# pvrohin/Structure-from-Motion-

Measured on AMD Instinct MI355X. Metric: BA LM-iterations/sec (+ RANSAC hypotheses/sec, final reproj RMSE vs ref), higher is better.
Workload: dtype f64; 1 GPU; cfg5: BA 200 cams / 500000 pts / 4000000 obs, Schur-complement LM, points sharded over 1 rank(s); parallelism=point-shard x1 + RCCL all-reduce of the reduced camera system

## Files before the change

### structure-from-motion-_amd/csrc/ba.hip

```cpp
#include <rccl/rccl.h>

#include <algorithm>
#include <chrono>
#include <condition_variable>
#include <deque>
#include <functional>
#include <mutex>
#include <thread>
#include <cmath>
#include <cstdio>
#include <cstdlib>
#include <cstring>
#include <memory>
#include <utility>
#include <numeric>
#include <vector>

#include "sfm_common.hpp"
#include "sfm_geom.hpp"
#include "host_pool.hpp"

struct LocalGroup {
    int nranks = 0;
    std::mutex mu;
// ... 30 lines not shown

__device__ __forceinline__ double clampd(double x) { return fmin(fmax(x, 1e-6), 1e32); }

__device__ __forceinline__ double wave_sum(double v) {
#pragma unroll
    for (int o = 32; o > 0; o >>= 1) v += __shfl_xor(v, o);
    return v;
}

template <int NV>
__device__ __forceinline__ void block_sum_store(double (&v)[NV], double *out) {
    __shared__ double red[PT_THREADS / 64][NV];
    const int lane = threadIdx.x & 63, w = threadIdx.x >> 6;
#pragma unroll
    for (int k = 0; k < NV; ++k) {
        const double s = wave_sum(v[k]);
        if (lane == 0) red[w][k] = s;
    }
    __syncthreads();
    if (threadIdx.x == 0) {
#pragma unroll
        for (int k = 0; k < NV; ++k) {
            double s = 0;
            for (int i = 0; i < PT_THREADS / 64; ++i) s += red[i][k];
            out[k] = s;
        }
    }
}

constexpr int GS_STRIDE = 32;
constexpr int GS_WORDS = 9 * GS_STRIDE;

template <int NV, int NT = PT_THREADS>
__device__ __forceinline__ void grid_sum_last(double (&v)[NV], double *partial, unsigned *counter, double *out) {
    __shared__ double red[NT / 64][NV];
    __shared__ int last;
    const int lane = threadIdx.x & 63, w = threadIdx.x >> 6;
    const unsigned nblk = gridDim.x;
#pragma unroll
    for (int k = 0; k < NV; ++k) {
        const double s = wave_sum(v[k]);
        if (lane == 0) red[w][k] = s;
    }
    __syncthreads();
    if (threadIdx.x == 0) {
#pragma unroll
        for (int k = 0; k < NV; ++k) {
            double s = 0;
            for (int i = 0; i < NT / 64; ++i) s += red[i][k];
            __hip_atomic_store(partial + (int64_t)NV * blockIdx.x + k, s, __ATOMIC_RELAXED, __HIP_MEMORY_SCOPE_AGENT);
        }
        asm volatile("s_waitcnt vmcnt(0)" ::: "memory");
        const unsigned g = blockIdx.x % 8, ng = (nblk - g + 7) / 8, ngroups = nblk < 8 ? nblk : 8;
        int l = 0;
        if (__hip_atomic_fetch_add(counter + GS_STRIDE * (1 + g), 1u, __ATOMIC_RELAXED, __HIP_MEMORY_SCOPE_AGENT) ==
            ng - 1)
            l = __hip_atomic_fetch_add(counter, 1u, __ATOMIC_RELAXED, __HIP_MEMORY_SCOPE_AGENT) == ngroups - 1;
        last = l;
    }
    __syncthreads();
    if (!last) return;
    __shared__ double tot[NV][NT];
    double s[NV];
#pragma unroll
    for (int k = 0; k < NV; ++k) s[k] = 0;
    constexpr int GS_BATCH = NV > 1 ? 8 : 16;
    for (unsigned b0 = threadIdx.x; b0 < nblk; b0 += GS_BATCH * NT) {
        double v16[NV][GS_BATCH];
#pragma unroll
        for (int u = 0; u < GS_BATCH; ++u) {
            const unsigned b = b0 + u * NT;
#pragma unroll
            for (int k = 0; k < NV; ++k)
                v16[k][u] = b < nblk ? __hip_atomic_load(partial + (int64_t)NV * b + k, __ATOMIC_RELAXED,
                                                         __HIP_MEMORY_SCOPE_AGENT)
                                     : 0.0;
        }
#pragma unroll
        for (int k = 0; k < NV; ++k)
#pragma unroll
            for (int u = 0; u < GS_BATCH; ++u) s[k] += v16[k][u];
    }
#pragma unroll
    for (int k = 0; k < NV; ++k) tot[k][threadIdx.x] = s[k];
    __syncthreads();
    for (int st = NT / 2; st > 0; st >>= 1) {
        if ((int)threadIdx.x < st)
#pragma unroll
            for (int k = 0; k < NV; ++k) tot[k][threadIdx.x] += tot[k][threadIdx.x + st];
        __syncthreads();
    }
    if (threadIdx.x < NV) out[threadIdx.x] = tot[threadIdx.x][0];
    if (threadIdx.x < 9) __hip_atomic_store(counter + GS_STRIDE * threadIdx.x, 0u, __ATOMIC_RELAXED, __HIP_MEMORY_SCOPE_AGENT);
}


__device__ __forceinline__ void obs_model(const double *__restrict__ Rt, const double *X, const double (&K)[9],
                                          double2 ob, double (&r)[2], double (&A)[2][3], double (&p)[3]) {
#pragma unroll
    for (int i = 0; i < 3; ++i) p[i] = Rt[3 * i] * X[0] + Rt[3 * i + 1] * X[1] + Rt[3 * i + 2] * X[2];
    const double xc0 = p[0] + Rt[9], xc1 = p[1] + Rt[10], xc2 = p[2] + Rt[11];
    double u[3];
#pragma unroll
    for (int i = 0; i < 3; ++i) u[i] = K[3 * i] * xc0 + K[3 * i + 1] * xc1 + K[3 * i + 2] * xc2;
    const double iw = 1.0 / (u[2] + 1e-8);
    const double pu = u[0] * iw, pv = u[1] * iw;
    r[0] = ob.x - pu;
    r[1] = ob.y - pv;
#pragma unroll
    for (int c = 0; c < 3; ++c) {
        A[0][c] = -(iw * K[c] - pu * iw * K[6 + c]);
        A[1][c] = -(iw * K[3 + c] - pv * iw * K[6 + c]);
    }
}

__device__ __forceinline__ void obs_Ap(const double *__restrict__ Rt, const double *X, const double (&K)[9],
                                       double (&A)[2][3], double (&p)[3]) {
#pragma unroll
    for (int i = 0; i < 3; ++i) p[i] = Rt[3 * i] * X[0] + Rt[3 * i + 1] * X[1] + Rt[3 * i + 2] * X[2];
    const double xc0 = p[0] + Rt[9], xc1 = p[1] + Rt[10], xc2 = p[2] + Rt[11];
    double u[3];
#pragma unroll
    for (int i = 0; i < 3; ++i) u[i] = K[3 * i] * xc0 + K[3 * i + 1] * xc1 + K[3 * i + 2] * xc2;
    const double iw = 1.0 / (u[2] + 1e-8);
    const double pu = u[0] * iw, pv = u[1] * iw;
#pragma unroll
// ... 2 lines not shown
        A[1][c] = -(iw * K[3 + c] - pv * iw * K[6 + c]);
    }
}

__device__ __forceinline__ void jc_of(const double (&A)[2][3], const double (&p)[3], double (&Jc)[2][6]) {
#pragma unroll
    for (int a = 0; a < 2; ++a) {
        Jc[a][0] = A[a][1] * (-p[2]) + A[a][2] * p[1];
        Jc[a][1] = A[a][0] * p[2] + A[a][2] * (-p[0]);
        Jc[a][2] = A[a][0] * (-p[1]) + A[a][1] * p[0];
        Jc[a][3] = A[a][0];
        Jc[a][4] = A[a][1];
        Jc[a][5] = A[a][2];
    }
}

__device__ __forceinline__ double obs_cost(const double *__restrict__ Rt, const double *X, const double (&K)[9],
                                           double2 ob) {
    double xc[3];
#pragma unroll
    for (int i = 0; i < 3; ++i) xc[i] = Rt[3 * i] * X[0] + Rt[3 * i + 1] * X[1] + Rt[3 * i + 2] * X[2] + Rt[9 + i];
    double u[3];
#pragma unroll
    for (int i = 0; i < 3; ++i) u[i] = K[3 * i] * xc[0] + K[3 * i + 1] * xc[1] + K[3 * i + 2] * xc[2];
    const double iw = 1.0 / (u[2] + 1e-8);
    const double r0 = ob.x - u[0] * iw, r1 = ob.y - u[1] * iw;
    return 0.5 * (r0 * r0 + r1 * r1);
}

struct Kmat {
    double k[9];
};

template <int G>
__global__ void __launch_bounds__(PT_THREADS) k_linearize(int64_t np_, const int32_t *__restrict__ pstart,
                                                          const int32_t *__restrict__ cam,
                                                          const double2 *__restrict__ obs, Kmat Km,
                                                          const double *__restrict__ Rt,
                                                          const double *__restrict__ X,
                                                          double *__restrict__ Vg, double *__restrict__ partial,
                                                          unsigned *__restrict__ counter, double *__restrict__ cost_out,
                                                          int want_cost, const int *__restrict__ gate, double gtol,
                                                          unsigned *__restrict__ nbig) {
    if (gate && !*gate) return;
    const int64_t gt = (int64_t)blockIdx.x * PT_THREADS + threadIdx.x;
    const int64_t p = gt / G;
    const int sub = (int)(gt % G);
    double K[9];
#pragma unroll
    for (int i = 0; i < 9; ++i) K[i] = Km.k[i];
    double acc[1] = {0.0};
    double V[6] = {0, 0, 0, 0, 0, 0}, g[3] = {0, 0, 0};
    if (p < np_) {
        double x[3] = {X[3 * p], X[3 * p + 1], X[3 * p + 2]};
        for (int32_t o = pstart[p] + sub; o < pstart[p + 1]; o += G) {
            const double *Rt_c = Rt + 12 * cam[o];
            double r[2], A[2][3], q[3];
            obs_model(Rt_c, x, K, obs[o], r, A, q);
            double Jp[2][3];
#pragma unroll
            for (int a = 0; a < 2; ++a)
#pragma unroll
                for (int c = 0; c < 3; ++c) Jp[a][c] = A[a][0] * Rt_c[c] + A[a][1] * Rt_c[3 + c] + A[a][2] * Rt_c[6 + c];
            acc[0] += 0.5 * (r[0] * r[0] + r[1] * r[1]);
            V[0] += Jp[0][0] * Jp[0][0] + Jp[1][0] * Jp[1][0];
            V[1] += Jp[0][0] * Jp[0][1] + Jp[1][0] * Jp[1][1];
            V[2] += Jp[0][0] * Jp[0][2] + Jp[1][0] * Jp[1][2];
            V[3] += Jp[0][1] * Jp[0][1] + Jp[1][1] * Jp[1][1];
            V[4] += Jp[0][1] * Jp[0][2] + Jp[1][1] * Jp[1][2];
            V[5] += Jp[0][2] * Jp[0][2] + Jp[1][2] * Jp[1][2];
#pragma unroll
            for (int i = 0; i < 3; ++i) g[i] += Jp[0][i] * r[0] + Jp[1][i] * r[1];
        }
    }
#pragma unroll
    for (int i = 0; i < 6; ++i) V[i] = group_sum<G>(V[i]);
#pragma unroll
    for (int i = 0; i < 3; ++i) g[i] = group_sum<G>(g[i]);
    if (p < np_ && sub == 0) {
        double *vg = Vg + 9 * p;
#pragma unroll
        for (int i = 0; i < 6; ++i) vg[i] = V[i];
#pragma unroll
        for (int i = 0; i < 3; ++i) vg[6 + i] = g[i];
    }
    if (gtol > 0.0) {
        int big = 0;
        if (p < np_ && sub == 0)
#pragma unroll
            for (int i = 0; i < 3; ++i) big += fabs(g[i]) >= gtol;
#pragma unroll
        for (int o = 32; o > 0; o >>= 1) big += __shfl_xor(big, o);
        if ((threadIdx.x & 63) == 0 && big) atomicAdd(nbig, (unsigned)big);
    }
    if (want_cost) grid_sum_last<1>(acc, partial, counter, cost_out);
}

constexpr int LIN_PRE = 4;
constexpr int LIN_CL_THREADS = 256;
#ifndef SFM_LIN_CAM_STRIDE
#define SFM_LIN_CAM_STRIDE 14
#endif
constexpr int LIN_CAM = SFM_LIN_CAM_STRIDE;
template <int G, int NT = LIN_CL_THREADS>
__global__ void __launch_bounds__(NT) k_linearize_cl(int64_t np_, int32_t nc, const int32_t *__restrict__ pstart,
                                                     const int32_t *__restrict__ cam, const double2 *__restrict__ obs,
                                                     Kmat Km, const double *__restrict__ Rt,
                                                     const double *__restrict__ X, double *__restrict__ Vg,
                                                     double *__restrict__ partial, unsigned *__restrict__ counter,
                                                     double *__restrict__ cost_out, int want_cost,
                                                     const int *__restrict__ gate, double gtol,
                                                     unsigned *__restrict__ nbig) {
    if (gate && !*gate) return;
    struct Pre {
        int32_t o0, o1;
        double x[3];
    };
    auto fetch = [&](int64_t g, Pre &P) {
        const int64_t p = g / G;
        const bool live = p < np_;
        P.o0 = live ? pstart[p] : 0;
        P.o1 = live ? pstart[p + 1] : 0;
#pragma unroll
        for (int i = 0; i < 3; ++i) P.x[i] = live ? X[3 * p + i] : 0.0;
    };
    const int64_t stride = (int64_t)gridDim.x * NT;
    Pre cur;
    fetch((int64_t)blockIdx.x * NT + threadIdx.x, cur);
    extern __shared__ __attribute__((aligned(16))) double lin_cam[];
#pragma unroll 4
    for (int i = threadIdx.x; i < 12 * nc; i += NT) lin_cam[LIN_CAM * (i / 12) + i % 12] = Rt[i];
    __syncthreads();
    double K[9];
#pragma unroll
    for (int i = 0; i < 9; ++i) K[i] = Km.k[i];
    double acc[1] = {0.0};
    int big = 0;
    for (int64_t gt = (int64_t)blockIdx.x * NT + threadIdx.x; gt / G < np_; gt += stride) {
        const int64_t p = gt / G;
        const int sub = (int)(gt % G);
        const int32_t o0 = cur.o0, o1 = cur.o1;
        int32_t cpre[LIN_PRE];
        double2 opre[LIN_PRE];
#pragma unroll
        for (int k = 0; k < LIN_PRE; ++k) {
            const int32_t o = o0 + sub + k * G;
            cpre[k] = o < o1 ? cam[o] : 0;
            opre[k] = o < o1 ? obs[o] : make_double2(0.0, 0.0);
        }
        Pre nxt;
        fetch(gt + stride, nxt);
        const double x[3] = {cur.x[0], cur.x[1], cur.x[2]};
        double V[6] = {0, 0, 0, 0, 0, 0}, g[3] = {0, 0, 0};
        auto add = [&](int32_t c, double2 ob) {
            const double *Rt_c = lin_cam + LIN_CAM * c;
            double r[2], A[2][3], q[3];
            obs_model(Rt_c, x, K, ob, r, A, q);
            double Jp[2][3];
#pragma unroll
            for (int a = 0; a < 2; ++a)
#pragma unroll
                for (int c2 = 0; c2 < 3; ++c2)
                    Jp[a][c2] = A[a][0] * Rt_c[c2] + A[a][1] * Rt_c[3 + c2] + A[a][2] * Rt_c[6 + c2];
            acc[0] += 0.5 * (r[0] * r[0] + r[1] * r[1]);
            V[0] += Jp[0][0] * Jp[0][0] + Jp[1][0] * Jp[1][0];
            V[1] += Jp[0][0] * Jp[0][1] + Jp[1][0] * Jp[1][1];
            V[2] += Jp[0][0] * Jp[0][2] + Jp[1][0] * Jp[1][2];
            V[3] += Jp[0][1] * Jp[0][1] + Jp[1][1] * Jp[1][1];
            V[4] += Jp[0][1] * Jp[0][2] + Jp[1][1] * Jp[1][2];
            V[5] += Jp[0][2] * Jp[0][2] + Jp[1][2] * Jp[1][2];
#pragma unroll
            for (int i = 0; i < 3; ++i) g[i] += Jp[0][i] * r[0] + Jp[1][i] * r[1];
        };
#pragma unroll
        for (int k = 0; k < LIN_PRE; ++k)
            if (o0 + sub + k * G < o1) add(cpre[k], opre[k]);
        for (int32_t o = o0 + sub + LIN_PRE * G; o < o1; o += G) add(cam[o], obs[o]);
#pragma unroll
        for (int i = 0; i < 6; ++i) V[i] = group_sum<G>(V[i]);
#pragma unroll
        for (int i = 0; i < 3; ++i) g[i] = group_sum<G>(g[i]);
        if (sub == 0) {
            double *vg = Vg + 9 * p;
#pragma unroll
            for (int i = 0; i < 6; ++i) vg[i] = V[i];
#pragma unroll
            for (int i = 0; i < 3; ++i) vg[6 + i] = g[i];
            if (gtol > 0.0)
#pragma unroll
                for (int i = 0; i < 3; ++i) big += fabs(g[i]) >= gtol;
        }
        cur = nxt;
    }
    if (gtol > 0.0) {
#pragma unroll
        for (int o = 32; o > 0; o >>= 1) big += __shfl_xor(big, o);
        if ((threadIdx.x & 63) == 0 && big) atomicAdd(nbig, (unsigned)big);
    }
    if (want_cost) grid_sum_last<1, NT>(acc, partial, counter, cost_out);
}

constexpr int OBS_THREADS = 256;

__global__ void __launch_bounds__(OBS_THREADS) k_point_prep(int64_t np_, const double *__restrict__ Vg,
                                                            const double *__restrict__ lam, double *__restrict__ Lq,
                                                            const int *__restrict__ gate) {
    if (gate && !*gate) return;
    __shared__ double buf[9 * OBS_THREADS];
    const int64_t p0 = (int64_t)blockIdx.x * OBS_THREADS;
    const int n9 = 9 * (int)(np_ - p0 < OBS_THREADS ? np_ - p0 : OBS_THREADS);
    const int t = threadIdx.x;
#pragma unroll
    for (int k = 0; k < 9; ++k)
        if (t + k * OBS_THREADS < n9) buf[t + k * OBS_THREADS] = Vg[9 * p0 + t + k * OBS_THREADS];
    __syncthreads();
    if (9 * t < n9) {
        const double lambda = *lam;
        double *vg = buf + 9 * t;
        const double v00 = vg[0] + lambda * clampd(vg[0]), v01 = vg[1], v02 = vg[2];
        const double v11 = vg[3] + lambda * clampd(vg[3]), v12 = vg[4];
// ... 1201 lines not shown
        chain_fetch<TB>(ob, A, nsp, nT - 2, lane);
        double acc = 0;
        lds_barrier();
        int kt = nT - 1;
        for (; kt >= 1; kt -= 2) {
            chain_step<TB>(oa, A, nsp, kt, x, acc, lane, li);
            chain_step<TB>(ob, A, nsp, kt - 1, x, acc, lane, li);
        }
        if (kt == 0) chain_step<TB>(oa, A, nsp, 0, x, acc, lane, li);
    } else {
        const int r = t - 64;
        double la[TB], lb[TB];
        rows_fetch<TB>(la, A, nsp, nT - 1, r);
        rows_fetch<TB>(lb, A, nsp, nT - 2, r);
        lds_barrier();
        int kt = nT - 1;
        for (; kt >= 1; kt -= 2) {
            rows_step<TB>(la, A, nsp, kt, x, r);
            rows_step<TB>(lb, A, nsp, kt - 1, x, r);
        }
        if (kt == 0) rows_step<TB>(la, A, nsp, 0, x, r);
    }
    lds_barrier();
    for (int i = t; i < nsp; i += SOLVE_THREADS) xg[i] = x[i];
    if (ct.nc > 0) {
        __shared__ double red[3][SOLVE_THREADS];
        camera_trial<SOLVE_THREADS>(ct.nc, x, ct.payload, ct.ns, *ct.lam, ct.Rt, ct.Rt_new, ct.cam_out, red);
    }
}

struct LMState {
    double lambda, nu, cost, cost0;
    int status, accepted, iters, done;
    int run_lin, run_step, accept_now, pad;
    double spec_lambda;
    int armed;
    int use_spec;
    int run_real;
    int run_spec;
};

struct HostLM {
    LMState st;
    int seq, pad[3];
};
constexpr int kHostRing = 4;

__global__ void __launch_bounds__(256) k_gather_cam_major(int64_t no, const int32_t *__restrict__ pt,
                                                         const double2 *__restrict__ obs, int32_t *cm_pt,
                                                         double2 *__restrict__ cm_obs) {
    const int64_t k = (int64_t)blockIdx.x * 256 + threadIdx.x;
    if (k >= no) return;
    const int32_t o = cm_pt[k];
    cm_pt[k] = pt[o];
    cm_obs[k] = obs[o];
}

__global__ void k_lm_reset(LMState *lm, double lambda0, int *bad) {
    lm->lambda = lambda0; lm->nu = 2.0; lm->cost = 0.0; lm->cost0 = 0.0;
    lm->status = 4; lm->accepted = 0; lm->iters = 0; lm->done = 0;
    lm->run_lin = 1; lm->run_step = 1; lm->accept_now = 0; lm->pad = 0;
    lm->spec_lambda = lambda0 * 2.0; lm->armed = 0; lm->use_spec = 0; lm->run_real = 1; lm->run_spec = 0;
    bad[0] = 0;
}

__global__ void k_lm_init(LMState *lm, const double *lin_cost) {
    const double c0 = *lin_cost;
    lm->cost = lm->cost0 = c0;
    if (!isfinite(c0)) {
        lm->status = 6;
        lm->done = 1;
        lm->run_step = 0;
        lm->run_lin = 0;
        lm->run_real = 0;
        lm->run_spec = 0;
    }
}

__device__ __forceinline__ LMState lm_decide(LMState lm, const double *__restrict__ h, int bad, int max_iterations,
                                             int fixed, double ftol, double ptol, double lambda0, int spec) {
#pragma clang fp contract(off)
    if (lm.done) { lm.accept_now = 0; return lm; }
    const bool built = (spec & 2) && lm.run_spec;
    const double built_lambda = lm.spec_lambda;
    const double cost = lm.cost;
    const double cost_new = h[0];
    const double model = 0.5 * (h[1] + h[4]);
    const double dnorm = sqrt(h[2] + h[5]), xnorm = sqrt(h[3] + h[6]);
    const double rho = (!bad && model > 0) ? (cost - cost_new) / model : -1.0;
    lm.iters += 1;
    int done = 0;
    if (!bad && isfinite(cost_new) && rho > 1e-3) {
        lm.accept_now = 1;
        const double dcost = cost - cost_new;
// ... 46 lines not shown
    __shared__ int big;
    if (threadIdx.x == 0) big = 0;
    __syncthreads();
    int b = 0;
    for (int i = threadIdx.x; i < 6 * nc; i += blockDim.x) b += fabs(gbuf[1 + i]) >= gtol;
    if (b) atomicAdd(&big, b);
    __syncthreads();
    if (threadIdx.x == 0 && big == 0 && gbuf[0] == 0.0) {
        lm->status = 2;
        lm->done = 1;
        lm->run_step = 0;
        lm->run_lin = 0;
        lm->run_real = 0;
        lm->run_spec = 0;
    }
}

__global__ void k_lm_step(const LMState *__restrict__ lm_in, LMState *__restrict__ lm_out,
                          const double *__restrict__ h, const int *__restrict__ bad_in, int *__restrict__ bad_next,
                          int max_iterations, int fixed, double ftol, double ptol, double lambda0, int64_t np_,
                          int32_t nc, double *__restrict__ X, const double *__restrict__ X2, double *__restrict__ Rt,
                          const double *__restrict__ Rt2, HostLM *__restrict__ ring, int seq, int spec) {
    const LMState lm = lm_decide(*lm_in, h, *bad_in, max_iterations, fixed, ftol, ptol, lambda0, spec);
    if (blockIdx.x == 0 && threadIdx.x == 0) {
        *lm_out = lm;
        *bad_next = 0;
        if (ring) {
            HostLM *r = ring + (seq - 1) % kHostRing;
            r->st = lm;
            __hip_atomic_store(&r->seq, seq, __ATOMIC_RELEASE, __HIP_MEMORY_SCOPE_SYSTEM);
        }
    }
    if (!lm.accept_now) return;
    const int64_t i0 = (int64_t)blockIdx.x * blockDim.x + threadIdx.x, st = (int64_t)gridDim.x * blockDim.x;
    for (int64_t i = i0; i < 3 * np_; i += st) X[i] = X2[i];
    for (int64_t i = i0; i < 12 * (int64_t)nc; i += st) Rt[i] = Rt2[i];
}

constexpr int LIN_CL_LANES = 2;
constexpr int LIN_LANES = 4;
constexpr int BS_LANES = 2;

template <int TB>
static int launch_cholesky_t(const double *payload, int32_t ns, const double *lam, double *A, int32_t nsp, double *b,
                             double *D, int *bad, hipStream_t s, const int *gate, const CamTrialArgs &ct,
                             const SlabSrc &src, int dpp) {
    const int nT = nsp / TB;
    for (int st = 0; st < nT; ++st) {
        const int T = nT - st;
        const int extra = st >= 1 || src.slab ? 1 : 0;
        hipLaunchKernelGGL(k_chol_col<TB>, dim3(T * (T + 1) / 2 + extra), dim3(256), 0, s, A, nsp, st, D, b, bad,
                           payload, ns, lam, gate, dpp, st == 0 ? src : SlabSrc{nullptr, nullptr, 0, 0},
                           const_cast<double *>(payload));
        SFM_HIP(hipGetLastError());
    }
    hipLaunchKernelGGL(k_chol_backsolve<TB>, dim3(1), dim3(SOLVE_THREADS), 0, s, A, nsp, b,
                       D + ((nT - 1) & 1) * TB * TB, ct, gate);
    SFM_HIP(hipGetLastError());
    return 0;
}

static int launch_cholesky(const double *payload, int32_t ns, const double *lam, double *A, int32_t nsp, double *b,
                           double *D, int *bad, hipStream_t s, int tb, const int *gate, const CamTrialArgs &ct,
                           const SlabSrc &src, int dpp) {
    return tb == 32 ? launch_cholesky_t<32>(payload, ns, lam, A, nsp, b, D, bad, s, gate, ct, src, dpp)
                    : launch_cholesky_t<16>(payload, ns, lam, A, nsp, b, D, bad, s, gate, ct, src, dpp);
// ... 203 lines not shown
    case gjr::TREG:
        hipLaunchKernelGGL((gjr::k_gjr_solve<gjr::TREG, 0>), dim3(g.nT), dim3(gjr::THREADS), gjr::DYN_LDS, s, a);
        break;
    default:
        hipLaunchKernelGGL((gjr::k_gjr_solve<gjr::TREG_L, gjr::TLDS_L>), dim3(g.nT), dim3(gjr::THREADS), gjr::DYN_LDS,
                           s, a);
        break;
    }
    SFM_HIP(hipGetLastError());
    return 0;
}

constexpr int BS_PRE = 6;
#ifndef SFM_BS_CAM_STRIDE
#define SFM_BS_CAM_STRIDE 30
#endif
constexpr int BS_CAM = SFM_BS_CAM_STRIDE;
static_assert(BS_CAM >= 30, "Rt 12 | Rt_new 12 | dc 6");
constexpr int BS_CAM_LDS_MAX = 64 * 1024;
template <int G, bool CL, int NT = PT_THREADS>
__global__ void __launch_bounds__(NT) k_backsub_trial(int64_t np_, int32_t nc, const int32_t *__restrict__ pstart,
                                                              const int32_t *__restrict__ cam,
                                                              const double2 *__restrict__ obs, Kmat Km,
                                                              const double *__restrict__ Vg,
                                                              const double *__restrict__ Lq_own,
                                                              const double *__restrict__ Lq_spec,
                                                              const int *__restrict__ use_spec,
                                                              const double *__restrict__ dc, const double *__restrict__ lam,
                                                              const double *__restrict__ Rt,
                                                              const double *__restrict__ Rt_new,
                                                              const double *__restrict__ X,
                                                              double *__restrict__ X_new, double *__restrict__ partial,
                                                              unsigned *__restrict__ counter, double *__restrict__ out,
                                                              const int *__restrict__ gate) {
    if (gate && !*gate) return;
    const double lambda = *lam;
    const double *__restrict__ Lq = use_spec && *use_spec ? Lq_spec : Lq_own;
    double K[9];
#pragma unroll
    for (int i = 0; i < 9; ++i) K[i] = Km.k[i];
    double acc[4] = {0, 0, 0, 0};
    struct Pre {
        int32_t o0, o1;
        double x[3], g[3], dg[3], l[6];
    };
    auto fetch = [&](int64_t gtn, Pre &P) {
        const int64_t p = gtn / G;
        const bool live = p < np_;
        P.o0 = live ? pstart[p] : 0;
        P.o1 = live ? pstart[p + 1] : 0;
        const double *vg = Vg + 9 * (live ? p : 0);
        const double *l = Lq + 9 * (live ? p : 0);
#pragma unroll
        for (int i = 0; i < 3; ++i) {
            P.x[i] = live ? X[3 * p + i] : 0.0;
            P.g[i] = vg[6 + i];
        }
        P.dg[0] = vg[0];
        P.dg[1] = vg[3];
        P.dg[2] = vg[5];
#pragma unroll
        for (int i = 0; i < 6; ++i) P.l[i] = l[i];
    };
    const int64_t stride = (int64_t)gridDim.x * NT;
    Pre cur;
    fetch((int64_t)blockIdx.x * NT + threadIdx.x, cur);
    extern __shared__ __attribute__((aligned(16))) double bs_cam[];
    if constexpr (CL) {
// ... 48 lines not shown
    };
#pragma unroll
    for (int k = 0; k < BS_PRE; ++k)
        if (o0 + sub + k * G < o1) wt_add(cpre[k]);
    for (int32_t o = o0 + sub + BS_PRE * G; o < o1; o += G) wt_add(cam[o]);
#pragma unroll
    for (int i = 0; i < 3; ++i) wt[i] = group_sum<G>(wt[i]);
    if (live) {
        const double rhs[3] = {-cur.g[0] - wt[0], -cur.g[1] - wt[1], -cur.g[2] - wt[2]};
        const double *l = cur.l;
        const double y0 = l[0] * rhs[0];
        const double y1 = l[1] * rhs[0] + l[3] * rhs[1];
        const double y2 = l[2] * rhs[0] + l[4] * rhs[1] + l[5] * rhs[2];
        const double dp[3] = {l[0] * y0 + l[1] * y1 + l[2] * y2, l[3] * y1 + l[4] * y2, l[5] * y2};
        double xn[3];
#pragma unroll
        for (int i = 0; i < 3; ++i) xn[i] = x[i] + dp[i];
        if (sub == 0) {
#pragma unroll
            for (int i = 0; i < 3; ++i) {
                X_new[3 * p + i] = xn[i];
                acc[1] += dp[i] * (lambda * clampd(cur.dg[i]) * dp[i] - cur.g[i]);
                acc[2] += dp[i] * dp[i];
                acc[3] += x[i] * x[i];
            }
        }
#pragma unroll
        for (int k = 0; k < BS_PRE; ++k)
            if (o0 + sub + k * G < o1) acc[0] += obs_cost(cRn + RS * cpre[k], xn, K, opre[k]);
        for (int32_t o = o0 + sub + BS_PRE * G; o < o1; o += G) acc[0] += obs_cost(cRn + RS * cam[o], xn, K, obs[o]);
    }
    cur = nxt;
    }
    grid_sum_last<4, NT>(acc, partial, counter, out);
}

static void h_rotvec_to_R(const double *w, double *R) {
    double th2 = w[0] * w[0] + w[1] * w[1] + w[2] * w[2];
    double th = std::sqrt(th2), a, b;
    if (th < 1e-6) {
        a = 1.0 - th2 / 6.0 + th2 * th2 / 120.0;
        b = 0.5 - th2 / 24.0 + th2 * th2 / 720.0;
    } else {
        a = std::sin(th) / th;
        b = (1.0 - std::cos(th)) / th2;
    }
    double x = w[0], y = w[1], z = w[2];
    R[0] = 1.0 - b * (y * y + z * z); R[1] = -a * z + b * x * y;       R[2] = a * y + b * x * z;
    R[3] = a * z + b * x * y;         R[4] = 1.0 - b * (x * x + z * z); R[5] = -a * x + b * y * z;
    R[6] = -a * y + b * x * z;        R[7] = a * x + b * y * z;         R[8] = 1.0 - b * (x * x + y * y);
}

static void h_R_to_rotvec(const double *R, double *w) {
    double tr = R[0] + R[4] + R[8], q[4];
    if (tr > R[0] && tr > R[4] && tr > R[8]) {
        q[3] = 1.0 + tr;
        q[0] = R[7] - R[5]; q[1] = R[2] - R[6]; q[2] = R[3] - R[1];
    } else {
        int i = (R[0] >= R[4] && R[0] >= R[8]) ? 0 : (R[4] >= R[8] ? 1 : 2);
        int j = (i + 1) % 3, k = (j + 1) % 3;
        q[i] = 1.0 - tr + 2.0 * R[i * 4];
        q[j] = R[j * 3 + i] + R[i * 3 + j];
        q[k] = R[k * 3 + i] + R[i * 3 + k];
        q[3] = R[k * 3 + j] - R[j * 3 + k];
    }
    double nq = std::sqrt(q[0] * q[0] + q[1] * q[1] + q[2] * q[2] + q[3] * q[3]);
    for (double &v : q) v /= nq;
// ... 1120 lines not shown
    uint32_t *d_sw_pairs = nullptr;
    int2 *d_sw_blkij = nullptr;
    double2 *d_obs = nullptr;
    double *d_Rt = nullptr, *d_Rt2 = nullptr, *d_X = nullptr, *d_X2 = nullptr;
    double *d_Vg = nullptr, *d_Lq = nullptr;
    double *d_payload = nullptr, *d_A = nullptr, *d_b = nullptr, *d_D = nullptr;
    double *d_partial = nullptr, *d_scal = nullptr;
    int *d_bad = nullptr;
    int *d_sw_err = nullptr;
    unsigned *d_count = nullptr;
    unsigned *d_nbig = nullptr;
    double *d_gbuf = nullptr;
    double gtol = 0.0;
    HostLM *h_ring = nullptr, *d_ring = nullptr;
    bool timing = false;
    int64_t payload_len = 0;
    int pt_blocks = 0;
    int bs_cl_blocks = 0;
    int lin_cl_blocks = 0;
    hipEvent_t ev[2 * T_NT] = {};
    hipEvent_t ev_it[2 * T_NT * kEvSlots] = {};
    LMState *d_lm = nullptr;
    GjPlan gjp;
    GjBufs gjb;
    int gj_epoch = 0;
    GjrPlan gjrp;
    GjrBufs gjrb;
    unsigned gjr_tag = 0;
    bool gjr_fold = false;
    hipEvent_t ev_solve = nullptr;
    bool spec_ok = false;
    bool spec_on = false;
    bool spec_armed = false;
    SweepSplit sp_split = {};
    int32_t sp_free_cus = 0;
    int32_t *d_sp_split_of = nullptr;
    double *d_sp_slab = nullptr;
    double *d_sp_Lq[2] = {nullptr, nullptr}, *d_sp_payload[2] = {nullptr, nullptr};
    SpecKit sk;
    bool sp_queued[kEvSlots] = {};
    double t_acc[T_NT] = {};
    int t_iters = 0;
    std::vector<std::pair<void *, size_t>> allocs;
    ~sfm_ba_problem() {
        (void)hipSetDevice(device);
        if (ev_solve && comm && comm->local) {
            std::lock_guard<std::mutex> lk(comm->local->solve_mu);
            if (comm->local->last_solve == ev_solve) comm->local->last_solve = nullptr;
        }
        const bool idle = stream && hipStreamSynchronize(stream) == hipSuccess &&
                          (!sk.stream || hipStreamSynchronize(sk.stream) == hipSuccess);
        for (auto &a : allocs) {
            if (idle) pool_free(a.first, a.second, device);
            else (void)hipFree(a.first);
        }
        if (stream && idle) {
            kit_release(*this);
            return;
        }
        (void)hipGetLastError();
        if (h_ring) (void)hipHostFree(h_ring);
        for (auto &e : ev)
            if (e) (void)hipEventDestroy(e);
        for (auto &e : ev_it)
            if (e) (void)hipEventDestroy(e);
        if (ev_solve) (void)hipEventDestroy(ev_solve);
// ... 888 lines not shown
    if (!p->comm) return 0;
    if (p->comm->local) return p->comm->nranks > 1 ? local_allreduce(p, buf, n) : 0;
    ncclResult_t r = ncclAllReduce(buf, buf, (size_t)n, ncclDouble, ncclSum, p->comm->comm, p->stream);
    if (r != ncclSuccess) {
        set_error("ncclAllReduce: %s", ncclGetErrorString(r));
        return SFM_ERR_COMM;
    }
    return 0;
}

static CamLinArgs camlin_args(const sfm_ba_problem *p, bool fused, const int *glin) {
    CamLinArgs a;
    a.items = fused ? p->d_fitems : p->d_items;
    a.wg_first = fused ? p->d_fwg_first : p->d_wg_first;
    a.cm_pt = p->d_cm_pt;
    a.cm_obs = p->d_cm_obs;
    a.X = p->d_X;
    a.Rt = p->d_Rt;
    a.Km = p->K;
    a.slab2 = p->d_slab2;
    a.blocks = fused ? p->d_fblocks : p->d_blocks;
    a.nblocks = p->ndiag_blocks;
    a.nwg = fused ? p->cl_fused_wg : p->ndiag_items;
    a.direct = !fused && p->ndiag_items == p->ndiag_blocks;
    a.camlin = p->d_camlin;
    a.counter = p->d_count + 2 * GS_WORDS;
    a.glin = glin;
    return a;
}

static int run_linearize(sfm_ba_problem *p, int par, int want_cost) {
    hipStream_t s = p->stream;
    const int *glin = &p->d_lm[par].run_lin;

    if (p->lin_cl_blocks > 0) {
        const int nb = std::max(1, std::min(ceil_div(p->np * LIN_CL_LANES, LIN_CL_THREADS), p->lin_cl_blocks));
        hipLaunchKernelGGL(k_linearize_cl<LIN_CL_LANES>, dim3(nb), dim3(LIN_CL_THREADS), (size_t)8 * LIN_CAM * p->nc, s,
                           p->np, p->nc, p->d_pstart, p->d_cam, p->d_obs, p->K, p->d_Rt, p->d_X, p->d_Vg, p->d_partial,
                           p->d_count, p->d_scal + 8, want_cost, glin, p->gtol, p->d_nbig);
        SFM_HIP(hipGetLastError());
        if (p->ndiag_items && !p->cl_fused) {
            const CamLinArgs cl = camlin_args(p, false, glin);
            hipLaunchKernelGGL(k_camera_lin<256>, dim3(p->ndiag_items), dim3(256), 0, s, cl);
            SFM_HIP(hipGetLastError());
        }
        return want_cost ? allreduce(p, p->d_scal + 8, 1) : 0;
    }
    const int nbl = std::max(1, ceil_div(p->np * LIN_LANES, PT_THREADS));
    hipLaunchKernelGGL(k_linearize<LIN_LANES>, dim3(nbl), dim3(PT_THREADS), 0, s, p->np, p->d_pstart, p->d_cam,
                       p->d_obs, p->K, p->d_Rt, p->d_X, p->d_Vg, p->d_partial, p->d_count, p->d_scal + 8, want_cost,
                       glin, p->gtol, p->d_nbig);
    SFM_HIP(hipGetLastError());
    if (p->ndiag_items && !p->cl_fused) {
        const CamLinArgs cl = camlin_args(p, false, glin);
        hipLaunchKernelGGL(k_camera_lin<256>, dim3(p->ndiag_items), dim3(256), 0, s, cl);
        SFM_HIP(hipGetLastError());
    }
    return want_cost ? allreduce(p, p->d_scal + 8, 1) : 0;
}

static int run_spec_chain(sfm_ba_problem *p, int par, int it, bool timed) {
    hipStream_t s2 = p->sk.stream;
    const int *gsp = &p->d_lm[par].run_spec;
    const double *lam = &p->d_lm[par].spec_lambda;
    double *Lq = p->d_sp_Lq[it & 1], *payload = p->d_sp_payload[it & 1];
    hipEvent_t *tm = p->sk.tm + 4 * (it % kEvSlots);
    if (timed) SFM_HIP(hipEventRecord(tm[0], s2));
    hipLaunchKernelGGL(k_point_prep, dim3(std::max(1, ceil_div(p->np, OBS_THREADS))), dim3(OBS_THREADS), 0, s2,
                       (int64_t)p->np, p->d_Vg, lam, Lq, gsp);
    SFM_HIP(hipGetLastError());
    if (timed) SFM_HIP(hipEventRecord(tm[1], s2));
    if (timed) SFM_HIP(hipEventRecord(tm[2], s2));
    const SweepSplit &sp = p->sp_split;
    const int nsweep = sp.S                ? sp.nfull + p->sw_nrange * sp.nsplit * sp.S
                       : p->sw_nrange < NXCD ? NXCD * ceil_div(p->sw_nspec, NXCD / p->sw_nrange)
                                             : NXCD * p->sw_nspec * ceil_div(p->sw_nrange, NXCD);
    auto sweep_k = p->sw_pinhole ? k_schur_sweep<1, true> : k_schur_sweep<1>;
    hipLaunchKernelGGL(sweep_k, dim3(nsweep), dim3(SW_THREADS), p->sw_lds_bytes, s2, p->sw_nspec, p->sw_nrange,
                       p->sw_nbd, p->sw_L, p->d_sw_rchunk, p->d_sw_nload, p->d_sw_goff, p->d_sw_groups,
                       p->d_sw_lanegrp, p->d_sw_scam, reinterpret_cast<const uint32_t *>(p->d_sw_list), p->d_sw_pairs,
                       p->d_sw_hdr, p->d_X, Lq, p->d_Rt, p->K, p->d_sp_slab, gsp, p->sw_debug, nsweep,
                       camlin_args(p, true, &p->d_lm[par].run_lin), (long long *)nullptr, p->d_sw_err, sp);
    SFM_HIP(hipGetLastError());
    hipLaunchKernelGGL(k_schur_finish, dim3(ceil_div(p->sw_nbd * ITEM_W, FIN_THREADS)), dim3(FIN_THREADS), 0, s2, p->ns,
                       p->sw_nbd, p->sw_nrange, p->d_sw_blkij, p->d_sp_slab, p->d_camlin, payload, gsp,
                       p->d_sp_split_of, sp);
    SFM_HIP(hipGetLastError());
    if (timed) SFM_HIP(hipEventRecord(tm[3], s2));
    SFM_HIP(hipEventRecord(p->sk.join[it % kSpecRing], s2));
    p->sp_queued[it % kEvSlots] = true;
    return 0;
}

static int run_step(sfm_ba_problem *p, hipEvent_t *ev, int par, int it) {
    hipStream_t s = p->stream;
    int rc;
    const bool timed = ev != nullptr;
    const int *gst = &p->d_lm[par].run_step;
    const int *greal = p->spec_on ? &p->d_lm[par].run_real : gst;
    const int *use_spec = p->spec_on ? &p->d_lm[par].use_spec : nullptr;
    const double *Lq_spec = p->spec_on ? p->d_sp_Lq[(it - 1) & 1] : nullptr;
    const double *pay_spec = p->spec_on ? p->d_sp_payload[(it - 1) & 1] : nullptr;
    const double *lam = &p->d_lm[par].lambda;
    int *bad = p->d_bad + par;
    if (timed) SFM_HIP(hipEventRecord(ev[2 * T_PREP], s));
    hipLaunchKernelGGL(k_point_prep, dim3(std::max(1, ceil_div(p->np, OBS_THREADS))), dim3(OBS_THREADS), 0, s, (int64_t)p->np,
                       p->d_Vg, lam, p->d_Lq, greal);
    SFM_HIP(hipGetLastError());
    if (timed) SFM_HIP(hipEventRecord(ev[2 * T_PREP + 1], s));
    if (timed) SFM_HIP(hipEventRecord(ev[2 * T_SCHUR], s));
    const int nsweep = p->sw_split.S       ? p->sw_split.nfull + NXCD * p->sw_split.nsplit * p->sw_split.S
                       : p->sw_nrange < NXCD ? NXCD * ceil_div(p->sw_nspec, NXCD / p->sw_nrange)
                                             : NXCD * p->sw_nspec * ceil_div(p->sw_nrange, NXCD);
    const bool fused = p->cl_fused && p->ndiag_items;
    auto sweep_k = p->sw_pinhole ? k_schur_sweep<1, true> : k_schur_sweep<1>;
    hipLaunchKernelGGL(sweep_k, dim3(nsweep + (fused ? p->cl_fused_wg : 0)), dim3(SW_THREADS),
                       p->sw_lds_bytes, s, p->sw_nspec, p->sw_nrange, p->sw_nbd, p->sw_L, p->d_sw_rchunk,
                       p->d_sw_nload, p->d_sw_goff, p->d_sw_groups, p->d_sw_lanegrp, p->d_sw_scam,
                       reinterpret_cast<const uint32_t *>(p->d_sw_list), p->d_sw_pairs, p->d_sw_hdr, p->d_X, p->d_Lq,
                       p->d_Rt, p->K, p->d_slab, greal, p->sw_debug, nsweep,
                       camlin_args(p, true, &p->d_lm[par].run_lin), sw_dbg_ptr(), p->d_sw_err, p->sw_split);
    SFM_HIP(hipGetLastError());
    const bool fin_fused = !p->comm && p->fin_fused && !p->gjp.cb && (!p->gjrp.ok() || p->gjr_fold);
    if (!fin_fused) {
        hipLaunchKernelGGL(k_schur_finish, dim3(ceil_div(p->sw_nbd * ITEM_W, FIN_THREADS)), dim3(FIN_THREADS), 0, s, p->ns, p->sw_nbd, p->sw_nrange,
                           p->d_sw_blkij, p->d_slab, p->d_camlin, p->d_payload, greal, p->d_sw_split_of, p->sw_split);
        SFM_HIP(hipGetLastError());
// ... 11 lines not shown
    const SlabSrc src = fin_fused ? SlabSrc{p->d_slab, p->d_camlin, p->sw_nbd, p->sw_nrange, p->sw_split, p->d_sw_split_of}
                                  : SlabSrc{nullptr, nullptr, 0, 0, {}, nullptr};
    if (p->gjp.cb || p->gjrp.ok()) {
        LocalGroup *lg = p->comm ? p->comm->local : nullptr;
        std::unique_lock<std::mutex> lk;
        if (lg) {
            lk = std::unique_lock<std::mutex>(lg->solve_mu);
            if (lg->last_solve) SFM_HIP(hipStreamWaitEvent(s, lg->last_solve, 0));
        }
        if (p->gjrp.ok()) {
            if ((rc = launch_gjr(p->gjrp, p->ns, p->d_payload, lam, p->gjrb, ++p->gjr_tag, p->d_b, bad, gst, ct, s,
                                 src, pay_spec, use_spec)))
                return rc;
        } else if ((rc = launch_gj(p->gjp, p->nT, p->ns, p->d_payload, lam, p->gjb, ++p->gj_epoch, p->d_b, bad,
                                   gst, ct, s, pay_spec, use_spec)))
            return rc;
        if (p->spec_armed && (rc = run_spec_chain(p, par, it, timed))) return rc;
        if (lg) {
            SFM_HIP(hipEventRecord(p->ev_solve, s));
            lg->last_solve = p->ev_solve;
        }
    } else if ((rc = launch_reduced_solve(p->ns, p->nsp, p->d_payload, lam, p->d_A, p->d_b, p->d_D, bad, s, p->tb,
                                          gst, ct, src, p->chol_dpp)))
        return rc;
    if (timed) SFM_HIP(hipEventRecord(ev[2 * T_SOLVE + 1], s));
    if (timed) SFM_HIP(hipEventRecord(ev[2 * T_TRIAL], s));
    const bool cl = p->bs_cl_blocks > 0;
    const int bst = cl ? 256 : PT_THREADS;
    const int nbb = std::max(1, std::min(ceil_div(p->np * BS_LANES, bst), cl ? p->bs_cl_blocks : 1024));
    const size_t cl_lds = cl ? (size_t)8 * BS_CAM * p->nc : 0;
    hipLaunchKernelGGL((cl ? k_backsub_trial<BS_LANES, true, 256> : k_backsub_trial<BS_LANES, false>), dim3(nbb),
                       dim3(bst), cl_lds, s, p->np, p->nc, p->d_pstart, p->d_cam, p->d_obs, p->K, p->d_Vg, p->d_Lq,
                       Lq_spec, use_spec, p->d_b, lam, p->d_Rt, p->d_Rt2, p->d_X, p->d_X2, p->d_partial, p->d_count + GS_WORDS, p->d_scal,
                       gst);
    SFM_HIP(hipGetLastError());
    if ((rc = allreduce(p, p->d_scal, 4))) return rc;
    if (timed) SFM_HIP(hipEventRecord(ev[2 * T_TRIAL + 1], s));
    if (p->spec_armed) SFM_HIP(hipStreamWaitEvent(s, p->sk.join[it % kSpecRing], 0));
    return 0;
}

static int wait_lm_state(sfm_ba_problem *p, int j) {
    const int *seq = &p->h_ring[j % kHostRing].seq;
    for (unsigned spin = 1;; ++spin) {
        if (__atomic_load_n(seq, __ATOMIC_ACQUIRE) == j + 1) return 0;
        if (spin % 256 == 0) {
            const hipError_t q = hipStreamQuery(p->stream);
            if (q == hipErrorNotReady) {
                std::this_thread::yield();
                continue;
            }
            if (__atomic_load_n(seq, __ATOMIC_ACQUIRE) == j + 1) return 0;
            set_error("LM iteration %d: state not published (%s)", j, hipGetErrorString(q));
            return SFM_ERR_HIP;
        }
    }
}

extern "C" int sfm_ba_set_timing(sfm_ba_problem *p, int on) {
    SFM_CHECK_ARG(p, "null pointer");
    p->timing = on != 0;
    return 0;
}

extern "C" int sfm_ba_solve(sfm_ba_problem *p, const sfm_ba_opts *o, sfm_ba_report *rep) {
    SFM_CHECK_ARG(p && o, "null pointer");
    SFM_CHECK_ARG(o->max_iterations >= 0, "max_iterations < 0");
    SFM_CHECK_ARG(o->gradient_tolerance >= 0.0, "gradient_tolerance < 0");
    SFM_HIP(hipSetDevice(p->device));
    p->gtol = o->gradient_tolerance;
    p->cl_fused = o->gradient_tolerance == 0.0 && env_int("SFM_CAMLIN_FUSED", 1) != 0;
    p->chol_dpp = env_int("SFM_CHOL_DPP", 1) != 0;
    p->fin_fused = env_int("SFM_FINISH_FUSED", 1) != 0;
    p->gjr_fold = env_int("SFM_GJR_FOLD", 0) != 0;
    p->spec_on = p->spec_ok && env_int("SFM_SPECULATE", 1) != 0 && o->gradient_tolerance == 0.0 &&
                 !(p->gjrp.ok() && p->gjr_fold);
    p->spec_armed = false;
    for (bool &q : p->sp_queued) q = false;
    (void)hipGetLastError();
    const auto t0 = std::chrono::steady_clock::now();
    for (double &t : p->t_acc) t = 0;
    p->t_iters = 0;
    hipStream_t s = p->stream;
    int rc;
    constexpr int depth = 2;
    static_assert(depth >= 1 && depth < kHostRing, "the host ring holds the iterations in flight");
    const bool timed = p->timing;
    for (int k = 0; k < kHostRing; ++k) __atomic_store_n(&p->h_ring[k].seq, 0, __ATOMIC_RELAXED);
    hipLaunchKernelGGL(k_lm_reset, dim3(1), dim3(1), 0, s, p->d_lm, o->initial_lambda, p->d_bad);
    SFM_HIP(hipGetLastError());
    if (p->gjp.cb) {
        SFM_HIP(hipMemsetAsync(p->gjb.err, 0, sizeof(int), s));
        SFM_HIP(hipMemsetAsync(p->gjb.arrive, 0, sizeof(unsigned), s));
    }
    if (p->gjrp.ok()) SFM_HIP(hipMemsetAsync(p->gjrb.err, 0, GjrBufs::ints * sizeof(int), s));
    SFM_HIP(hipMemsetAsync(p->d_sw_err, 0, sizeof(int), s));
    auto account = [&](int j) {
        const hipEvent_t *e = p->ev_it + (size_t)(j % kEvSlots) * 2 * T_NT;
        for (int k = 0; k < T_NT; ++k) {
            float ms = 0;
            if (hipEventElapsedTime(&ms, e[2 * k], e[2 * k + 1]) == hipSuccess) p->t_acc[k] += ms;
        }
        if (p->sp_queued[j % kEvSlots]) {
            const hipEvent_t *tm = p->sk.tm + 4 * (j % kEvSlots);
            float ms = 0;
            if (hipEventElapsedTime(&ms, tm[0], tm[1]) == hipSuccess) p->t_acc[T_PREP] += ms;
            if (hipEventElapsedTime(&ms, tm[2], tm[3]) == hipSuccess) p->t_acc[T_SCHUR] += ms;
            p->sp_queued[j % kEvSlots] = false;
        }
        p->t_iters++;
    };
    const int64_t nacc = std::max<int64_t>(3 * p->np, 12 * (int64_t)p->nc);
    int it = 0;
    for (; it < o->max_iterations; ++it) {
        if (it >= depth) {
            const int j = it - depth;
            if ((rc = wait_lm_state(p, j))) return rc;
            const LMState &st = p->h_ring[j % kHostRing].st;
            if (timed && st.iters == j + 1) account(j);
            if (st.done) break;
            if (p->spec_on && !p->spec_armed && st.armed) {
                if ((rc = p->sk.make(timed))) return rc;
                p->spec_armed = true;
            }
        }
        hipEvent_t *ev = timed ? p->ev_it + (size_t)(it % kEvSlots) * 2 * T_NT : nullptr;
        if (timed) SFM_HIP(hipEventRecord(ev[2 * T_LIN], s));
        const int par = it & 1;
        if ((rc = run_linearize(p, par, it == 0))) return rc;
        if (timed) SFM_HIP(hipEventRecord(ev[2 * T_LIN + 1], s));
        if (it == 0) {
            hipLaunchKernelGGL(k_lm_init, dim3(1), dim3(1), 0, s, p->d_lm, p->d_scal + 8);
            SFM_HIP(hipGetLastError());
        }
        if (o->gradient_tolerance > 0.0) {
            const int *glin = &p->d_lm[par].run_lin;
            hipLaunchKernelGGL(k_gtol_pack, dim3(1), dim3(256), 0, s, p->nc, p->d_camlin, p->d_nbig, p->d_gbuf, glin);
            SFM_HIP(hipGetLastError());
            if ((rc = allreduce(p, p->d_gbuf, 6 * (int64_t)p->nc + 1))) return rc;
            hipLaunchKernelGGL(k_gtol_check, dim3(1), dim3(256), 0, s, p->nc, o->gradient_tolerance, p->d_gbuf,
                               p->d_lm + par, glin);
            SFM_HIP(hipGetLastError());
        }
        if ((rc = run_step(p, ev, par, it))) return rc;
        hipLaunchKernelGGL(k_lm_step, dim3(std::min(ceil_div(nacc, 256), 512)), dim3(256), 0, s, p->d_lm + par,
                           p->d_lm + (par ^ 1),
                           p->d_scal, p->d_bad + par, p->d_bad + (par ^ 1), o->max_iterations, o->fixed_iterations,
                           o->function_tolerance, o->parameter_tolerance, o->initial_lambda, p->np, p->nc, p->d_X,
                           p->d_X2, p->d_Rt, p->d_Rt2, p->d_ring, it + 1, (p->spec_on ? 1 : 0) | (p->spec_armed ? 2 : 0));
        SFM_HIP(hipGetLastError());
    }
    LMState h{};
    int gj_err = 0;
    SFM_HIP(hipMemcpyAsync(&h, p->d_lm + (it & 1), sizeof h, hipMemcpyDeviceToHost, s));
    if (p->gjp.cb) SFM_HIP(hipMemcpyAsync(&gj_err, p->gjb.err, sizeof gj_err, hipMemcpyDeviceToHost, s));
    if (p->gjrp.ok()) SFM_HIP(hipMemcpyAsync(&gj_err, p->gjrb.err, sizeof gj_err, hipMemcpyDeviceToHost, s));
    int sw_err = 0;
    SFM_HIP(hipMemcpyAsync(&sw_err, p->d_sw_err, sizeof sw_err, hipMemcpyDeviceToHost, s));
    SFM_HIP(hipStreamSynchronize(s));
    if (sw_err) {
        set_error("Schur sweep: a workgroup timed out waiting for a chunk hand-off");
        return SFM_ERR_HIP;
    }
    if (gj_err) {
        set_error("reduced camera solve: a workgroup of the persistent solve timed out waiting for a panel");
        return SFM_ERR_HIP;
    }
    if (timed)
        for (int j = std::max(0, it - depth); j < it && j < h.iters; ++j)
            if (p->h_ring[j % kHostRing].st.iters == j + 1) account(j);
    const auto t1 = std::chrono::steady_clock::now();
    if (rep) {
        rep->iterations = h.iters;
        rep->accepted = h.accepted;
        rep->status = h.status;
        rep->n_ranks = p->comm ? p->comm->nranks : 1;
        rep->cost0 = h.cost0;
        rep->cost = h.cost;
        rep->t_loop_ms = std::chrono::duration<double, std::milli>(t1 - t0).count();
        rep->lambda = h.lambda;
    }
    return 0;
// ... 227 lines not shown
```

Baseline: 2271 LM-iterations/s.

## Fold LM accept decision into trial kernel and defer parameter copy to linearize

The LM accept/reject decision now runs in the last workgroup of the backsubstitution trial kernel, using the grid-reduced totals. This removes the separate k_lm_step launch on single-rank runs. The copy of accepted X2/Rt2 into X/Rt is deferred: the next linearize reads directly from the trial buffers and writes them back while it runs, and a final move kernel covers the last iteration. This saves a kernel launch and a full pass over the point array each iteration, but adds a move_pending state flag and extra writes inside linearize.

```diff
diff --git a/structure-from-motion-_amd/csrc/ba.hip b/structure-from-motion-_amd/csrc/ba.hip
--- a/structure-from-motion-_amd/csrc/ba.hip
+++ b/structure-from-motion-_amd/csrc/ba.hip
@@ -86,7 +86,8 @@
 constexpr int GS_WORDS = 9 * GS_STRIDE;
 
 template <int NV, int NT = PT_THREADS>
-__device__ __forceinline__ void grid_sum_last(double (&v)[NV], double *partial, unsigned *counter, double *out) {
+__device__ __forceinline__ bool grid_sum_last(double (&v)[NV], double *partial, unsigned *counter, double *out,
+                                              double *tot_out = nullptr) {
     __shared__ double red[NT / 64][NV];
     __shared__ int last;
     const int lane = threadIdx.x & 63, w = threadIdx.x >> 6;
@@ -113,7 +114,7 @@
         last = l;
     }
     __syncthreads();
-    if (!last) return;
+    if (!last) return false;
     __shared__ double tot[NV][NT];
     double s[NV];
 #pragma unroll
@@ -146,6 +147,10 @@
     }
     if (threadIdx.x < NV) out[threadIdx.x] = tot[threadIdx.x][0];
     if (threadIdx.x < 9) __hip_atomic_store(counter + GS_STRIDE * threadIdx.x, 0u, __ATOMIC_RELAXED, __HIP_MEMORY_SCOPE_AGENT);
+    if (tot_out)
+#pragma unroll
+        for (int k = 0; k < NV; ++k) tot_out[k] = tot[k][0];
+    return true;
 }
 
 
@@ -214,20 +219,29 @@
     double k[9];
 };
 
+struct MoveSrc {
+    const int *pending;
+    const double *X2, *Rt2;
+    int32_t nc;
+};
+
 template <int G>
 __global__ void __launch_bounds__(PT_THREADS) k_linearize(int64_t np_, const int32_t *__restrict__ pstart,
                                                           const int32_t *__restrict__ cam,
                                                           const double2 *__restrict__ obs, Kmat Km,
-                                                          const double *__restrict__ Rt,
-                                                          const double *__restrict__ X,
+                                                          double *Rt_cur, double *X_cur,
                                                           double *__restrict__ Vg, double *__restrict__ partial,
                                                           unsigned *__restrict__ counter, double *__restrict__ cost_out,
                                                           int want_cost, const int *__restrict__ gate, double gtol,
-                                                          unsigned *__restrict__ nbig) {
+                                                          unsigned *__restrict__ nbig, const MoveSrc mv) {
     if (gate && !*gate) return;
     const int64_t gt = (int64_t)blockIdx.x * PT_THREADS + threadIdx.x;
     const int64_t p = gt / G;
     const int sub = (int)(gt % G);
+    const bool moved = mv.pending && *mv.pending;
+    const double *const Rt = moved ? mv.Rt2 : Rt_cur, *const X = moved ? mv.X2 : X_cur;
+    if (moved && blockIdx.x == 0)
+        for (int i = threadIdx.x; i < 12 * mv.nc; i += PT_THREADS) Rt_cur[i] = Rt[i];
     double K[9];
 #pragma unroll
     for (int i = 0; i < 9; ++i) K[i] = Km.k[i];
@@ -265,6 +279,9 @@
         for (int i = 0; i < 6; ++i) vg[i] = V[i];
 #pragma unroll
         for (int i = 0; i < 3; ++i) vg[6 + i] = g[i];
+        if (moved)
+#pragma unroll
+            for (int i = 0; i < 3; ++i) X_cur[3 * p + i] = X[3 * p + i];
     }
     if (gtol > 0.0) {
         int big = 0;
@@ -287,13 +304,15 @@
 template <int G, int NT = LIN_CL_THREADS>
 __global__ void __launch_bounds__(NT) k_linearize_cl(int64_t np_, int32_t nc, const int32_t *__restrict__ pstart,
                                                      const int32_t *__restrict__ cam, const double2 *__restrict__ obs,
-                                                     Kmat Km, const double *__restrict__ Rt,
-                                                     const double *__restrict__ X, double *__restrict__ Vg,
+                                                     Kmat Km, double *Rt_cur, double *X_cur,
+                                                     double *__restrict__ Vg,
                                                      double *__restrict__ partial, unsigned *__restrict__ counter,
                                                      double *__restrict__ cost_out, int want_cost,
                                                      const int *__restrict__ gate, double gtol,
-                                                     unsigned *__restrict__ nbig) {
+                                                     unsigned *__restrict__ nbig, const MoveSrc mv) {
     if (gate && !*gate) return;
+    const bool moved = mv.pending && *mv.pending;
+    const double *const Rt = moved ? mv.Rt2 : Rt_cur, *const X = moved ? mv.X2 : X_cur;
     struct Pre {
         int32_t o0, o1;
         double x[3];
@@ -312,6 +331,8 @@
     extern __shared__ __attribute__((aligned(16))) double lin_cam[];
 #pragma unroll 4
     for (int i = threadIdx.x; i < 12 * nc; i += NT) lin_cam[LIN_CAM * (i / 12) + i % 12] = Rt[i];
+    if (moved && blockIdx.x == 0)
+        for (int i = threadIdx.x; i < 12 * nc; i += NT) Rt_cur[i] = Rt[i];
     __syncthreads();
     double K[9];
 #pragma unroll
@@ -368,6 +389,9 @@
             for (int i = 0; i < 6; ++i) vg[i] = V[i];
 #pragma unroll
             for (int i = 0; i < 3; ++i) vg[6 + i] = g[i];
+            if (moved)
+#pragma unroll
+                for (int i = 0; i < 3; ++i) X_cur[3 * p + i] = x[i];
             if (gtol > 0.0)
 #pragma unroll
                 for (int i = 0; i < 3; ++i) big += fabs(g[i]) >= gtol;
@@ -1635,7 +1659,8 @@
 struct LMState {
     double lambda, nu, cost, cost0;
     int status, accepted, iters, done;
-    int run_lin, run_step, accept_now, pad;
+    int run_lin, run_step, accept_now;
+    int move_pending;
     double spec_lambda;
     int armed;
     int use_spec;
@@ -1662,7 +1687,7 @@
 __global__ void k_lm_reset(LMState *lm, double lambda0, int *bad) {
     lm->lambda = lambda0; lm->nu = 2.0; lm->cost = 0.0; lm->cost0 = 0.0;
     lm->status = 4; lm->accepted = 0; lm->iters = 0; lm->done = 0;
-    lm->run_lin = 1; lm->run_step = 1; lm->accept_now = 0; lm->pad = 0;
+    lm->run_lin = 1; lm->run_step = 1; lm->accept_now = 0; lm->move_pending = 0;
     lm->spec_lambda = lambda0 * 2.0; lm->armed = 0; lm->use_spec = 0; lm->run_real = 1; lm->run_spec = 0;
     bad[0] = 0;
 }
@@ -1775,6 +1800,44 @@
         }
     }
     if (!lm.accept_now) return;
+    const int64_t i0 = (int64_t)blockIdx.x * blockDim.x + threadIdx.x, st = (int64_t)gridDim.x * blockDim.x;
+    for (int64_t i = i0; i < 3 * np_; i += st) X[i] = X2[i];
+    for (int64_t i = i0; i < 12 * (int64_t)nc; i += st) Rt[i] = Rt2[i];
+}
+
+struct LmFold {
+    const LMState *lm_in;
+    LMState *lm_out;
+    const int *bad_in;
+    int *bad_next;
+    const double *scal;
+    HostLM *ring;
+    double ftol, ptol, lambda0;
+    int max_iterations, fixed, seq, spec;
+};
+
+__device__ __forceinline__ void lm_fold_decide(const LmFold &f, const double *tot) {
+    const LMState old = *f.lm_in;
+    double h[7];
+#pragma unroll
+    for (int k = 0; k < 4; ++k) h[k] = tot ? tot[k] : 0.0;
+#pragma unroll
+    for (int k = 4; k < 7; ++k) h[k] = f.scal[k];
+    LMState lm = lm_decide(old, h, *f.bad_in, f.max_iterations, f.fixed, f.ftol, f.ptol, f.lambda0, f.spec);
+    lm.move_pending = lm.accept_now || (old.move_pending && !old.run_lin);
+    *f.lm_out = lm;
+    *f.bad_next = 0;
+    if (f.ring) {
+        HostLM *r = f.ring + (f.seq - 1) % kHostRing;
+        r->st = lm;
+        __hip_atomic_store(&r->seq, f.seq, __ATOMIC_RELEASE, __HIP_MEMORY_SCOPE_SYSTEM);
+    }
+}
+
+__global__ void __launch_bounds__(256) k_lm_move(const LMState *__restrict__ lm, int64_t np_, int32_t nc,
+                                                 double *__restrict__ X, const double *__restrict__ X2,
+                                                 double *__restrict__ Rt, const double *__restrict__ Rt2) {
+    if (!lm->move_pending) return;
     const int64_t i0 = (int64_t)blockIdx.x * blockDim.x + threadIdx.x, st = (int64_t)gridDim.x * blockDim.x;
     for (int64_t i = i0; i < 3 * np_; i += st) X[i] = X2[i];
     for (int64_t i = i0; i < 12 * (int64_t)nc; i += st) Rt[i] = Rt2[i];
@@ -2044,8 +2107,11 @@
                                                               const double *__restrict__ X,
                                                               double *__restrict__ X_new, double *__restrict__ partial,
                                                               unsigned *__restrict__ counter, double *__restrict__ out,
-                                                              const int *__restrict__ gate) {
-    if (gate && !*gate) return;
+                                                              const int *__restrict__ gate, const LmFold fold) {
+    if (gate && !*gate) {
+        if (fold.lm_out && blockIdx.x == 0 && threadIdx.x == 0) lm_fold_decide(fold, nullptr);
+        return;
+    }
     const double lambda = *lam;
     const double *__restrict__ Lq = use_spec && *use_spec ? Lq_spec : Lq_own;
     double K[9];
@@ -2160,7 +2226,9 @@
     }
     cur = nxt;
     }
-    grid_sum_last<4, NT>(acc, partial, counter, out);
+    double tot[4];
+    if (!grid_sum_last<4, NT>(acc, partial, counter, out, tot)) return;
+    if (fold.lm_out && threadIdx.x == 0) lm_fold_decide(fold, tot);
 }
 
 static void h_rotvec_to_R(const double *w, double *R) {
@@ -3347,6 +3415,7 @@
     bool spec_ok = false;
     bool spec_on = false;
     bool spec_armed = false;
+    bool lm_fold = false;
     SweepSplit sp_split = {};
     int32_t sp_free_cus = 0;
     int32_t *d_sp_split_of = nullptr;
@@ -4301,12 +4370,13 @@
 static int run_linearize(sfm_ba_problem *p, int par, int want_cost) {
     hipStream_t s = p->stream;
     const int *glin = &p->d_lm[par].run_lin;
+    const MoveSrc mv = {p->lm_fold ? &p->d_lm[par].move_pending : nullptr, p->d_X2, p->d_Rt2, p->nc};
 
     if (p->lin_cl_blocks > 0) {
         const int nb = std::max(1, std::min(ceil_div(p->np * LIN_CL_LANES, LIN_CL_THREADS), p->lin_cl_blocks));
         hipLaunchKernelGGL(k_linearize_cl<LIN_CL_LANES>, dim3(nb), dim3(LIN_CL_THREADS), (size_t)8 * LIN_CAM * p->nc, s,
                            p->np, p->nc, p->d_pstart, p->d_cam, p->d_obs, p->K, p->d_Rt, p->d_X, p->d_Vg, p->d_partial,
-                           p->d_count, p->d_scal + 8, want_cost, glin, p->gtol, p->d_nbig);
+                           p->d_count, p->d_scal + 8, want_cost, glin, p->gtol, p->d_nbig, mv);
         SFM_HIP(hipGetLastError());
         if (p->ndiag_items && !p->cl_fused) {
             const CamLinArgs cl = camlin_args(p, false, glin);
@@ -4318,7 +4388,7 @@
     const int nbl = std::max(1, ceil_div(p->np * LIN_LANES, PT_THREADS));
     hipLaunchKernelGGL(k_linearize<LIN_LANES>, dim3(nbl), dim3(PT_THREADS), 0, s, p->np, p->d_pstart, p->d_cam,
                        p->d_obs, p->K, p->d_Rt, p->d_X, p->d_Vg, p->d_partial, p->d_count, p->d_scal + 8, want_cost,
-                       glin, p->gtol, p->d_nbig);
+                       glin, p->gtol, p->d_nbig, mv);
     SFM_HIP(hipGetLastError());
     if (p->ndiag_items && !p->cl_fused) {
         const CamLinArgs cl = camlin_args(p, false, glin);
@@ -4361,7 +4431,7 @@
     return 0;
 }
 
-static int run_step(sfm_ba_problem *p, hipEvent_t *ev, int par, int it) {
+static int run_step(sfm_ba_problem *p, hipEvent_t *ev, int par, int it, const LmFold &fold) {
     hipStream_t s = p->stream;
     int rc;
     const bool timed = ev != nullptr;
@@ -4439,7 +4509,7 @@
     hipLaunchKernelGGL((cl ? k_backsub_trial<BS_LANES, true, 256> : k_backsub_trial<BS_LANES, false>), dim3(nbb),
                        dim3(bst), cl_lds, s, p->np, p->nc, p->d_pstart, p->d_cam, p->d_obs, p->K, p->d_Vg, p->d_Lq,
                        Lq_spec, use_spec, p->d_b, lam, p->d_Rt, p->d_Rt2, p->d_X, p->d_X2, p->d_partial, p->d_count + GS_WORDS, p->d_scal,
-                       gst);
+                       gst, fold);
     SFM_HIP(hipGetLastError());
     if ((rc = allreduce(p, p->d_scal, 4))) return rc;
     if (timed) SFM_HIP(hipEventRecord(ev[2 * T_TRIAL + 1], s));
@@ -4483,6 +4553,7 @@
     p->spec_on = p->spec_ok && env_int("SFM_SPECULATE", 1) != 0 && o->gradient_tolerance == 0.0 &&
                  !(p->gjrp.ok() && p->gjr_fold);
     p->spec_armed = false;
+    p->lm_fold = env_int("SFM_LM_FOLD", 1) != 0 && !p->comm && o->gradient_tolerance == 0.0;
     for (bool &q : p->sp_queued) q = false;
     (void)hipGetLastError();
     const auto t0 = std::chrono::steady_clock::now();
@@ -4549,12 +4620,32 @@
                                p->d_lm + par, glin);
             SFM_HIP(hipGetLastError());
         }
-        if ((rc = run_step(p, ev, par, it))) return rc;
+        const int spec = (p->spec_on ? 1 : 0) | (p->spec_armed ? 2 : 0);
+        const LmFold fold = {p->d_lm + par,
+                             p->lm_fold ? p->d_lm + (par ^ 1) : nullptr,
+                             p->d_bad + par,
+                             p->d_bad + (par ^ 1),
+                             p->d_scal,
+                             p->d_ring,
+                             o->function_tolerance,
+                             o->parameter_tolerance,
+                             o->initial_lambda,
+                             o->max_iterations,
+                             o->fixed_iterations,
+                             it + 1,
+                             spec};
+        if ((rc = run_step(p, ev, par, it, fold))) return rc;
+        if (p->lm_fold) continue;
         hipLaunchKernelGGL(k_lm_step, dim3(std::min(ceil_div(nacc, 256), 512)), dim3(256), 0, s, p->d_lm + par,
                            p->d_lm + (par ^ 1),
                            p->d_scal, p->d_bad + par, p->d_bad + (par ^ 1), o->max_iterations, o->fixed_iterations,
                            o->function_tolerance, o->parameter_tolerance, o->initial_lambda, p->np, p->nc, p->d_X,
-                           p->d_X2, p->d_Rt, p->d_Rt2, p->d_ring, it + 1, (p->spec_on ? 1 : 0) | (p->spec_armed ? 2 : 0));
+                           p->d_X2, p->d_Rt, p->d_Rt2, p->d_ring, it + 1, spec);
+        SFM_HIP(hipGetLastError());
+    }
+    if (p->lm_fold) {
+        hipLaunchKernelGGL(k_lm_move, dim3(std::min(ceil_div(nacc, 256), 512)), dim3(256), 0, s, p->d_lm + (it & 1),
+                           (int64_t)p->np, p->nc, p->d_X, p->d_X2, p->d_Rt, p->d_Rt2);
         SFM_HIP(hipGetLastError());
     }
     LMState h{};
```

Measured after the change: 2283 LM-iterations/s, median of 6. About the same (+0.5%).
